# Kiripiro/leaffliction

Measured on AMD Instinct MI355X. Metric: 224x224 images/sec train, higher is better.
Workload: dtype f32; 1 GPU; leaf_cnn base train step (configs[1]: img 224, batch 256/GPU, fp32, 8 classes, AdamW+clipnorm+EMA, in-model augmentation); per_gpu_batch=256, global_batch=256, img_size=224, parallelism=dp1

## Files before the change

leaffliction_amd/csrc/lf_conv.hip:

```cpp
#include <type_traits>

#include "lf_common.h"

namespace {

typedef float f32x16 __attribute__((ext_vector_type(16)));
typedef float f32x4 __attribute__((ext_vector_type(4)));

constexpr int kThreads = 256;

typedef float lf_f4 __attribute__((ext_vector_type(4)));
constexpr unsigned kBufOob = 0xffffffffu;
__device__ __forceinline__ __amdgpu_buffer_rsrc_t buf_rsrc(const float* base, unsigned bytes) {
    return __builtin_amdgcn_make_buffer_rsrc(const_cast<float*>(base), 0, bytes, 0x00020000);
}
__device__ __forceinline__ float4 buf_load4(__amdgpu_buffer_rsrc_t r, unsigned off) {
    const lf_f4 v = __builtin_bit_cast(lf_f4, __builtin_amdgcn_raw_buffer_load_b128(r, off, 0, 0));
    return make_float4(v.x, v.y, v.z, v.w);
}
__device__ __forceinline__ float buf_load1(__amdgpu_buffer_rsrc_t r, unsigned off) {
    return __builtin_bit_cast(float, __builtin_amdgcn_raw_buffer_load_b32(r, off, 0, 0));
}

struct ConvArgs {
    const float* x;
    const float* w;
    const float* wino_u;
    float* y;
    const float* in_scale;
    const float* in_shift;
    int n, cin, cout, h, wd;
    int tiles_x, tiles_y;
    int in_relu;
    int accumulate;
    int vec_ok;
    int stack;
    float* stat_part;
    const float* stat_pivot;
    long long stat_tiles;
    const float* stat_mask_y;
    const float* mask_scale;
    const float* mask_shift;
    int mask_relu;
};

using lf::half_sum32;
using lf::pro_apply;
using lf::row_sum16;

__device__ __forceinline__ void wino_filter(const float (&g)[9], float (&u)[16]) {
    float t[4][3];
#pragma unroll
    for (int c = 0; c < 3; ++c) {
        const float s = g[c] + g[6 + c];
        t[0][c] = g[c];
        t[1][c] = (s + g[3 + c]) * 0.5f;
        t[2][c] = (s - g[3 + c]) * 0.5f;
        t[3][c] = g[6 + c];
    }
#pragma unroll
    for (int r = 0; r < 4; ++r) {
        const float s = t[r][0] + t[r][2];
        u[r * 4 + 0] = t[r][0];
        u[r * 4 + 1] = (s + t[r][1]) * 0.5f;
        u[r * 4 + 2] = (s - t[r][1]) * 0.5f;
        u[r * 4 + 3] = t[r][2];
    }
}
__device__ __forceinline__ void wino_input(const float (&d)[16], float (&v)[16]) {
    float t[16];
#pragma unroll
    for (int c = 0; c < 4; ++c) {
        t[0 + c] = d[0 + c] - d[8 + c];
        t[4 + c] = d[4 + c] + d[8 + c];
        t[8 + c] = d[8 + c] - d[4 + c];
        t[12 + c] = d[4 + c] - d[12 + c];
    }
#pragma unroll
    for (int r = 0; r < 4; ++r) {
        v[r * 4 + 0] = t[r * 4 + 0] - t[r * 4 + 2];
        v[r * 4 + 1] = t[r * 4 + 1] + t[r * 4 + 2];
        v[r * 4 + 2] = t[r * 4 + 2] - t[r * 4 + 1];
        v[r * 4 + 3] = t[r * 4 + 1] - t[r * 4 + 3];
    }
}
__device__ __forceinline__ void wino_output(const float (&m)[16], float (&y)[4]) {
    float b[2][4];
#pragma unroll
    for (int c = 0; c < 4; ++c) {
        b[0][c] = m[0 + c] + m[4 + c] + m[8 + c];
        b[1][c] = m[4 + c] - m[8 + c] - m[12 + c];
    }
#pragma unroll
    for (int r = 0; r < 2; ++r) {
        y[r * 2 + 0] = b[r][0] + b[r][1] + b[r][2];
        y[r * 2 + 1] = b[r][1] - b[r][2] - b[r][3];
    }
}

constexpr int kMaxProC = 512;

template <int TW, int TH, int HALO, bool STK>
struct ConvTile {
    int bz, by, tile;
    int tx0, ty0, n;
    int imgA, gyA0, ra;
    bool imgA_ok, imgB_ok;

    __device__ __forceinline__ explicit ConvTile(const ConvArgs& p) {
        const lf::Block3 b = lf::xcd_block3();
        bz = b.z;
        by = b.y;
        tile = b.x;
        tx0 = (tile % p.tiles_x) * TW;
        ty0 = (tile / p.tiles_x) * TH;
        n = bz * p.stack;
        imgA = ty0 / p.h;
        gyA0 = ty0 - imgA * p.h;
        ra = min(TH, p.h - gyA0);
        imgA_ok = imgA < p.stack && n + imgA < p.n;
        imgB_ok = STK && imgA + 1 < p.stack && n + imgA + 1 < p.n;
    }

    __device__ __forceinline__ bool patch_row(int py, int h, int& img, int& gy) const {
        if (py < ra + 2 * HALO) {
            img = imgA;
            gy = gyA0 - HALO + py;
            return imgA_ok && gy >= 0 && gy < h;
        }
        img = imgA + 1;
        gy = py - (ra + 2 * HALO) - HALO;
        return imgB_ok && ra < TH && gy >= 0 && gy < h && gy < TH - ra + HALO;
    }
};

template <int TW, int TH, int HALO, bool STK, int kKC>
struct PatchStage {
    static constexpr int PW = TW + 2 * HALO, PH = TH + 2 * HALO + (STK ? 2 * HALO : 0), PP = PW * PH;
    static constexpr int TW4 = TW / 4;
    static constexpr int NVI = kKC * PH * TW4, IPT = (NVI + kThreads - 1) / kThreads;
    static constexpr int NHI = kKC * PH * 2 * HALO, HPT = (NHI + kThreads - 1) / kThreads;
    static_assert(TW % 4 == 0, "float4 patch rows");

    size_t hw;
    float4 pv[IPT];
    float ph[HPT > 0 ? HPT : 1];
    unsigned pg[IPT], pl[IPT];
    unsigned hg[HPT > 0 ? HPT : 1], hl[HPT > 0 ? HPT : 1];
    unsigned okmask = 0;

    __device__ __forceinline__ PatchStage(const ConvArgs& p, const ConvTile<TW, TH, HALO, STK>& t, float* lsc, int tid) {
        if (p.in_scale != nullptr) {
            for (int c = tid; c < p.cin && c < kMaxProC; c += kThreads) {
                lsc[c] = p.in_scale[c];
                lsc[kMaxProC + c] = p.in_shift[c];
            }
        }
        hw = (size_t)p.h * p.wd;
        const unsigned uhw = (unsigned)hw;
#pragma unroll
        for (int i = 0; i < IPT; ++i) {
            const int e = tid + i * kThreads;
            const int kc = e / (PH * TW4), rem = e - kc * (PH * TW4);
            const int py = rem / TW4, slot = rem - py * TW4;
            int img, gy;
            const bool ok = t.patch_row(py, p.h, img, gy) && e < NVI;
            pg[i] = ok ? 4u * ((unsigned)(img * p.cin + kc) * uhw + (unsigned)gy * (unsigned)p.wd + (unsigned)(t.tx0 + 4 * slot)) : kBufOob;
            pl[i] = (unsigned)(kc * PP + py * PW + HALO + 4 * slot) | ((unsigned)kc << 16);
            okmask |= (ok ? 1u : 0u) << i;
        }
#pragma unroll
        for (int i = 0; i < HPT; ++i) {
            const int e = tid + i * kThreads;
            const int kc = e / (PH * 2), rem = e - kc * (PH * 2);
            const int py = rem >> 1, side = rem & 1;
            const int gx = side ? t.tx0 + TW : t.tx0 - 1;
            int img, gy;
            const bool ok = t.patch_row(py, p.h, img, gy) && e < NHI && gx >= 0 && gx < p.wd;
            hg[i] = ok ? 4u * ((unsigned)(img * p.cin + kc) * uhw + (unsigned)gy * (unsigned)p.wd + (unsigned)gx) : kBufOob;
            hl[i] = (unsigned)(kc * PP + py * PW + (side ? PW - 1 : 0)) | ((unsigned)kc << 16);
            okmask |= (ok ? 1u : 0u) << (16 + i);
        }
    }

    __device__ __forceinline__ void load(const ConvArgs& p, const float* xin, int c0) {
        const __amdgpu_buffer_rsrc_t rx = buf_rsrc(
            xin + (size_t)c0 * hw,
            4u * (unsigned)((STK ? (p.stack - 1) * p.cin : 0) + min(kKC, p.cin - c0)) * (unsigned)hw);
#pragma unroll
        for (int i = 0; i < IPT; ++i) pv[i] = buf_load4(rx, pg[i]);
#pragma unroll
        for (int i = 0; i < HPT; ++i) ph[i] = buf_load1(rx, hg[i]);
    }

    __device__ __forceinline__ void store(const ConvArgs& p, float* lp, const float* lsc, int c0, int tid) const {
        const bool pro = p.in_scale != nullptr;
        auto pro_sc = [&](int c) { return c < kMaxProC ? lsc[c] : p.in_scale[c]; };
        auto pro_sh = [&](int c) { return c < kMaxProC ? lsc[kMaxProC + c] : p.in_shift[c]; };
#pragma unroll
        for (int i = 0; i < IPT; ++i) {
            if (tid + i * kThreads < NVI) {
                const int kc = (int)(pl[i] >> 16);
                float4 v = pv[i];
                if (pro && (okmask >> i & 1u)) {
                    const float sc = pro_sc(c0 + kc), sh = pro_sh(c0 + kc);
                    v.x = pro_apply(v.x, sc, sh, p.in_relu);
                    v.y = pro_apply(v.y, sc, sh, p.in_relu);
                    v.z = pro_apply(v.z, sc, sh, p.in_relu);
                    v.w = pro_apply(v.w, sc, sh, p.in_relu);
                }
                float* dst = lp + (pl[i] & 0xffffu);
                dst[0] = v.x;
                dst[1] = v.y;
                dst[2] = v.z;
                dst[3] = v.w;
            }
        }
#pragma unroll
        for (int i = 0; i < HPT; ++i) {
            if (tid + i * kThreads < NHI) {
                const int kc = (int)(hl[i] >> 16);
                float v = ph[i];
                if (pro && (okmask >> (16 + i) & 1u))
                    v = pro_apply(v, pro_sc(c0 + kc), pro_sh(c0 + kc), p.in_relu);
                lp[hl[i] & 0xffffu] = v;
            }
        }
    }

    static __device__ __forceinline__ void stage_scalar(const ConvArgs& p, float* lp, const float* xin,
                                                        int tx0, int ty0, int c0, int tid) {
        constexpr int SLOTS = PP <= 64 ? 64 : (PP <= 128 ? 128 : 256);
        constexpr int G = kThreads / SLOTS;
        constexpr int ROUNDS = (PP + SLOTS - 1) / SLOTS;
        const int slot = tid % SLOTS, grp = tid / SLOTS;
        const size_t hw = (size_t)p.h * p.wd;
        const unsigned uhw = (unsigned)hw;
        const bool pro = p.in_scale != nullptr;
#pragma unroll
        for (int r = 0; r < ROUNDS; ++r) {
            const int pos = slot + r * SLOTS;
            if (pos < PP) {
                const int py = pos / PW, px = pos - py * PW;
                const int gy = ty0 + py - HALO, gx = tx0 + px - HALO;
                const bool inb = gy >= 0 && gy < p.h && gx >= 0 && gx < p.wd;
                const unsigned goff = inb ? (unsigned)gy * (unsigned)p.wd + (unsigned)gx : 0u;
#pragma unroll 4
                for (int kc = grp; kc < kKC; kc += G) {
                    const int c = c0 + kc;
                    float v = 0.f;
                    if (inb && c < p.cin) {
                        v = xin[(unsigned)c * uhw + goff];
                        if (pro) v = pro_apply(v, p.in_scale[c], p.in_shift[c], p.in_relu);
                    }
                    lp[kc * PP + pos] = v;
                }
            }
        }
    }
};

template <int WPX, int CT>
__device__ __forceinline__ void write_stat_part(const ConvArgs& p, const float* red, int bz, int tile, int co0,
                                                int tid) {
    __syncthreads();
    lf::write_stat_part<WPX, CT>(p.stat_part, p.stat_tiles, p.cout, (long long)bz * (p.tiles_x * p.tiles_y) + tile,
                                 co0, red, tid, kThreads);
}

template <int TAPS, int TW, int TH, int WCO, int MB, int WPX, int NB, int kKC, bool STK = false>
__global__ __launch_bounds__(kThreads, (MB * NB * 16 <= 32 ? 3 : 2))
void conv_mfma_kernel(ConvArgs p) {
    constexpr int NPB = TW * TH / 32;
    static_assert(TW * TH % 32 == 0, "tile must be whole 32-pixel blocks");
    static_assert(WCO * WPX == 4 && WPX * NB == NPB, "wave decomposition");
    constexpr int CT = 32 * WCO * MB;
    constexpr int HALO = TAPS == 9 ? 1 : 0;
    using Patch = PatchStage<TW, TH, HALO, STK, kKC>;
    constexpr int PW = Patch::PW, PP = Patch::PP;
    constexpr int PATCH = kKC * PP;
    constexpr int WSZ = kKC * TAPS * CT;
    static_assert(PATCH % 4 == 0, "16-byte aligned weight region");
    constexpr int CT4 = CT / 4, NWI = kKC * TAPS * CT4, WPT = (NWI + kThreads - 1) / kThreads;

    __shared__ __attribute__((aligned(16))) float lds[PATCH + WSZ];
    __shared__ float lsc[2 * kMaxProC];
    float* lp = lds;
    float* lw = lds + PATCH;

    const int tid = threadIdx.x, lane = tid & 63, wid = tid >> 6;
    const int wave_co = wid % WCO, wave_px = wid / WCO;
    const ConvTile<TW, TH, HALO, STK> t(p);
    const int co0 = t.by * CT;
    const size_t hw = (size_t)p.h * p.wd;
    const unsigned uhw = (unsigned)hw;
    const float* xin = p.x + (size_t)t.n * p.cin * hw;

    const int khalf = lane >> 5, j = lane & 31;
    int bbase[NB];
#pragma unroll
    for (int nb = 0; nb < NB; ++nb) {
        const int f = (wave_px * NB + nb) * 32 + j;
        const int r = f / TW, prow = (STK && r >= t.ra) ? r + 2 * HALO : r;
        bbase[nb] = khalf * PP + prow * PW + (f % TW);
    }
    const int abase = khalf * TAPS * CT + wave_co * MB * 32 + j;

    f32x16 acc[MB][NB];
#pragma unroll
    for (int m = 0; m < MB; ++m)
#pragma unroll
        for (int nb = 0; nb < NB; ++nb)
#pragma unroll
            for (int r = 0; r < 16; ++r) acc[m][nb][r] = 0.f;

    auto compute_chunk = [&]() {
#pragma unroll 2
        for (int cp = 0; cp < kKC / 2; ++cp) {
            const float* lwc = lw + abase + 2 * cp * TAPS * CT;
            const float* lpc = lp + 2 * cp * PP;
#pragma unroll
            for (int tap = 0; tap < TAPS; ++tap) {
                const int dy = TAPS == 9 ? tap / 3 : 0, dx = TAPS == 9 ? tap % 3 : 0;
                float a[MB], b[NB];
#pragma unroll
                for (int m = 0; m < MB; ++m) a[m] = lwc[tap * CT + m * 32];
#pragma unroll
                for (int nb = 0; nb < NB; ++nb) b[nb] = lpc[bbase[nb] + dy * PW + dx];
#pragma unroll
                for (int m = 0; m < MB; ++m)
#pragma unroll
                    for (int nb = 0; nb < NB; ++nb)
                        acc[m][nb] = __builtin_amdgcn_mfma_f32_32x32x2f32(a[m], b[nb], acc[m][nb], 0, 0, 0);
            }
        }
    };

    const int nchunks = (p.cin + kKC - 1) / kKC;
    const bool vec = p.vec_ok && (t.tx0 + TW <= p.wd);

    if (vec) {
        float4 wv[WPT];
        constexpr bool kPrefetchW = MB * NB * 16 <= 64;
        Patch patch(p, t, lsc, tid);
        unsigned wg[WPT];
#pragma unroll
        for (int i = 0; i < WPT; ++i) {
            const int e = tid + i * kThreads;
            const int row = e / CT4, col = (e - row * CT4) * 4;
            wg[i] = (e < NWI && co0 + col < p.cout) ? 4u * ((unsigned)row * (unsigned)p.cout + (unsigned)(co0 + col)) : kBufOob;
        }
        auto load_weights = [&](int c0) {
            const __amdgpu_buffer_rsrc_t rw =
                buf_rsrc(p.w + (size_t)c0 * TAPS * p.cout,
                         4u * (unsigned)(min(kKC, p.cin - c0) * TAPS) * (unsigned)p.cout);
#pragma unroll
            for (int i = 0; i < WPT; ++i) wv[i] = buf_load4(rw, wg[i]);
        };
        auto store_chunk = [&](int c0) {
            if (!kPrefetchW) load_weights(c0);
            patch.store(p, lp, lsc, c0, tid);
#pragma unroll
            for (int i = 0; i < WPT; ++i) {
                const int e = tid + i * kThreads;
                if (e < NWI) reinterpret_cast<float4*>(lw)[e] = wv[i];
            }
        };
        patch.load(p, xin, 0);
        if (kPrefetchW) load_weights(0);
        for (int ch = 0; ch < nchunks; ++ch) {
            __syncthreads();
            store_chunk(ch * kKC);
            __syncthreads();
            if (ch + 1 < nchunks) {
                patch.load(p, xin, (ch + 1) * kKC);
                if (kPrefetchW) load_weights((ch + 1) * kKC);
            }
            compute_chunk();
        }
    } else {
        constexpr int WROWS = kKC * TAPS, RPP = kThreads / CT;
        const int wcol = tid % CT, wrow0 = tid / CT;
        const bool wcol_ok = co0 + wcol < p.cout;
        for (int ch = 0; ch < nchunks; ++ch) {
            const int c0 = ch * kKC;
            __syncthreads();
            Patch::stage_scalar(p, lp, xin, t.tx0, t.ty0, c0, tid);
            const int wvalid = (p.cin - c0) * TAPS;
#pragma unroll 4
            for (int row = wrow0; row < WROWS; row += RPP) {
                float v = 0.f;
                if (wcol_ok && row < wvalid)
                    v = p.w[((unsigned)c0 * TAPS + row) * (unsigned)p.cout + (unsigned)(co0 + wcol)];
                lw[row * CT + wcol] = v;
            }
            __syncthreads();
            compute_chunk();
        }
    }

    float* yout = p.y + (size_t)t.n * p.cout * hw;
    const bool stats = p.stat_part != nullptr, masked = p.stat_mask_y != nullptr;
    float* red = lds;
    static_assert(WPX * CT * 2 <= PATCH + WSZ, "stat scratch must fit the staging LDS");
    if (stats) __syncthreads();
    const float* my = masked ? p.stat_mask_y + (size_t)t.n * p.cout * hw : nullptr;
    constexpr int RG = TAPS == 1 ? (NB <= 2 ? 4 : 1) : (NB <= 2 ? 16 : 4);
    bool pix_ok[NB];
    unsigned pixc[NB];
#pragma unroll
    for (int nb = 0; nb < NB; ++nb) {
        const int f = (wave_px * NB + nb) * 32 + j;
        const int r = f / TW, ox = t.tx0 + f % TW;
        const bool in_a = r < t.ra;
        const int oy = in_a ? t.gyA0 + r : r - t.ra;
        pix_ok[nb] = (in_a ? t.imgA_ok : t.imgB_ok) && oy < p.h && ox < p.wd;
        pixc[nb] = pix_ok[nb] ? (unsigned)((in_a ? t.imgA : t.imgA + 1) * p.cout) * uhw +
                                    (unsigned)oy * (unsigned)p.wd + (unsigned)ox
                              : 0u;
    }
#pragma unroll
    for (int m = 0; m < MB; ++m) {
#pragma unroll
        for (int rg = 0; rg < 16; rg += RG) {
            float oldv[RG][NB], yv[RG][NB];
            if (p.accumulate) {
#pragma unroll
                for (int rr = 0; rr < RG; ++rr) {
                    const int r = rg + rr;
                    const int co = co0 + (wave_co * MB + m) * 32 + 4 * khalf + (r & 3) + 8 * (r >> 2);
                    const float* src = yout + (size_t)min(co, p.cout - 1) * hw;
#pragma unroll
                    for (int nb = 0; nb < NB; ++nb) oldv[rr][nb] = src[pixc[nb]];
                }
            }
            if (masked) {
#pragma unroll
                for (int rr = 0; rr < RG; ++rr) {
                    const int r = rg + rr;
                    const int co = co0 + (wave_co * MB + m) * 32 + 4 * khalf + (r & 3) + 8 * (r >> 2);
                    const float* src = my + (size_t)min(co, p.cout - 1) * hw;
#pragma unroll
                    for (int nb = 0; nb < NB; ++nb) yv[rr][nb] = src[pixc[nb]];
                }
            }
#pragma unroll
            for (int rr = 0; rr < RG; ++rr) {
                const int r = rg + rr;
                const int cl = (wave_co * MB + m) * 32 + 4 * khalf + (r & 3) + 8 * (r >> 2);
                const int co = co0 + cl;
                const bool co_ok = co < p.cout;
                float* dst = yout + (size_t)co * hw;
#pragma unroll
                for (int nb = 0; nb < NB; ++nb) {
                    if (p.accumulate) acc[m][nb][r] += oldv[rr][nb];
                    if (co_ok && pix_ok[nb])
                        dst[pixc[nb]] = acc[m][nb][r];
                }
                if (!stats) continue;
                float s1 = 0.f, s2 = 0.f;
                if (!masked) {
                    const float pv = (p.stat_pivot != nullptr && co_ok) ? p.stat_pivot[co] : 0.f;
#pragma unroll
                    for (int nb = 0; nb < NB; ++nb)
                        lf::stat_accumulate(acc[m][nb][r], pix_ok[nb], false, pv, 0.f, 0.f, 0.f, 0, s1, s2);
                } else {
                    const float msc = p.mask_scale[min(co, p.cout - 1)], msh = p.mask_shift[min(co, p.cout - 1)];
#pragma unroll
                    for (int nb = 0; nb < NB; ++nb)
                        lf::stat_accumulate(acc[m][nb][r], co_ok && pix_ok[nb], true, 0.f, yv[rr][nb], msc, msh,
                                            p.mask_relu, s1, s2);
                }
                s1 = half_sum32(s1);
                s2 = half_sum32(s2);
                if (j == 31) {
                    red[(wave_px * CT + cl) * 2] = s1;
                    red[(wave_px * CT + cl) * 2 + 1] = s2;
                }
            }
        }
    }
    if (stats) write_stat_part<WPX, CT>(p, red, t.bz, t.tile, co0, tid);
}

template <int TW, int TH, int MB, int NB, bool STK>
__global__ __launch_bounds__(kThreads, 2)
void conv_wino_kernel(ConvArgs p) {
    constexpr int kKC = 8, WPX = 4;
    constexpr int TXN = TW / 2, NT = TXN * (TH / 2);
    static_assert(TH % 2 == 0, "F(2x2,3x3): even tile");
    static_assert(WPX * NB * 16 >= NT, "wave decomposition");
    constexpr int CT = 16 * MB;
    constexpr int kUP = 20;
    using Patch = PatchStage<TW, TH, 1, STK, kKC>;
    constexpr int PW = Patch::PW, PP = Patch::PP;
    constexpr int PATCH = kKC * PP;
    constexpr int WSZ = kKC * CT * kUP;
    static_assert(PATCH % 4 == 0, "16-byte aligned U region");

    __shared__ __attribute__((aligned(16))) float lds[PATCH + WSZ];
    __shared__ float lsc[2 * kMaxProC];
    float* lp = lds;
    float* lw = lds + PATCH;

    const int tid = threadIdx.x, lane = tid & 63, wave_px = tid >> 6;
    const ConvTile<TW, TH, 1, STK> t(p);
    const int co0 = t.by * CT;
    const size_t hw = (size_t)p.h * p.wd;
    const unsigned uhw = (unsigned)hw;
    const float* xin = p.x + (size_t)t.n * p.cin * hw;

    const int wq = lane >> 4, wl = lane & 15;
    int vbase[NB];
    const int ubase = (wq * CT + wl) * kUP;
    f32x4 wacc[MB][NB][16];
#pragma unroll
    for (int nb = 0; nb < NB; ++nb) {
        const int tt = min((wave_px * NB + nb) * 16 + wl, NT - 1);
        const int r0 = 2 * (tt / TXN), prow = (STK && r0 >= t.ra) ? r0 + 2 : r0;
        vbase[nb] = wq * PP + prow * PW + 2 * (tt % TXN);
    }
#pragma unroll
    for (int m = 0; m < MB; ++m)
#pragma unroll
        for (int nb = 0; nb < NB; ++nb)
#pragma unroll
            for (int q = 0; q < 16; ++q) wacc[m][nb][q] = f32x4{0.f, 0.f, 0.f, 0.f};

    auto compute_chunk = [&]() {
#pragma unroll
        for (int s = 0; s < kKC / 4; ++s) {
            float u[MB][16];
#pragma unroll
            for (int m = 0; m < MB; ++m) {
                const float4* us = reinterpret_cast<const float4*>(lw + ubase + (4 * s * CT + m * 16) * kUP);
#pragma unroll
                for (int q4 = 0; q4 < 4; ++q4) {
                    const float4 v4 = us[q4];
                    u[m][4 * q4 + 0] = v4.x;
                    u[m][4 * q4 + 1] = v4.y;
                    u[m][4 * q4 + 2] = v4.z;
                    u[m][4 * q4 + 3] = v4.w;
                }
            }
#pragma unroll
            for (int nb = 0; nb < NB; ++nb) {
                const float* src = lp + vbase[nb] + 4 * s * PP;
                float d[16], v[16];
#pragma unroll
                for (int r = 0; r < 4; ++r) {
                    const float2 lo = *reinterpret_cast<const float2*>(src + r * PW);
                    const float2 hi = *reinterpret_cast<const float2*>(src + r * PW + 2);
                    d[r * 4 + 0] = lo.x;
                    d[r * 4 + 1] = lo.y;
                    d[r * 4 + 2] = hi.x;
                    d[r * 4 + 3] = hi.y;
                }
                wino_input(d, v);
#pragma unroll
                for (int m = 0; m < MB; ++m)
#pragma unroll
                    for (int q = 0; q < 16; ++q)
                        wacc[m][nb][q] = __builtin_amdgcn_mfma_f32_16x16x4f32(u[m][q], v[q], wacc[m][nb][q], 0, 0, 0);
            }
        }
    };

    constexpr int KSTEP = kThreads / (4 * CT), UPT = kKC / KSTEP;
    static_assert(kThreads % (4 * CT) == 0 && kKC % KSTEP == 0, "whole channels per pass");
    const int ukc = tid / (4 * CT), uco = (tid >> 2) % CT, uq4 = tid & 3;
    const unsigned ustep = 64u * KSTEP * (unsigned)p.cout;
    const unsigned ugo = co0 + uco < p.cout ? 4u * (((unsigned)ukc * (unsigned)p.cout + (unsigned)(co0 + uco)) * 16u + 4u * (unsigned)uq4) : 0x80000000u;
    float* const ulds = lw + (ukc * CT + uco) * kUP + 4 * uq4;
    float4 uv[UPT];
    auto load_u = [&](int c0) {
        const __amdgpu_buffer_rsrc_t ru =
            buf_rsrc(p.wino_u + (size_t)c0 * p.cout * 16, 64u * (unsigned)min(kKC, p.cin - c0) * (unsigned)p.cout);
#pragma unroll
        for (int i = 0; i < UPT; ++i) uv[i] = buf_load4(ru, ugo + (unsigned)i * ustep);
    };
    auto store_u = [&]() {
#pragma unroll
        for (int i = 0; i < UPT; ++i) *reinterpret_cast<float4*>(ulds + i * KSTEP * CT * kUP) = uv[i];
    };

    const int nchunks = (p.cin + kKC - 1) / kKC;
    const bool vec = p.vec_ok && (t.tx0 + TW <= p.wd);

    if (vec) {
        Patch patch(p, t, lsc, tid);
        patch.load(p, xin, 0);
        for (int ch = 0; ch < nchunks; ++ch) {
            __syncthreads();
            load_u(ch * kKC);
            patch.store(p, lp, lsc, ch * kKC, tid);
            store_u();
            __syncthreads();
            if (ch + 1 < nchunks) patch.load(p, xin, (ch + 1) * kKC);
            compute_chunk();
        }
    } else {
        for (int ch = 0; ch < nchunks; ++ch) {
            const int c0 = ch * kKC;
            __syncthreads();
            Patch::stage_scalar(p, lp, xin, t.tx0, t.ty0, c0, tid);
            load_u(c0);
            store_u();
            __syncthreads();
            compute_chunk();
        }
    }

    float* yout = p.y + (size_t)t.n * p.cout * hw;
    const bool stats = p.stat_part != nullptr, masked = p.stat_mask_y != nullptr;
    float* red = lds;
    static_assert(WPX * CT * 2 <= PATCH + WSZ, "stat scratch must fit the staging LDS");
    if (stats) __syncthreads();
    const float* my = masked ? p.stat_mask_y + (size_t)t.n * p.cout * hw : nullptr;
    const bool y2 = (p.wd & 1) == 0 && (reinterpret_cast<size_t>(p.y) & 7) == 0;
    bool pok[NB][4];
    unsigned pofs[NB][4];
#pragma unroll
    for (int nb = 0; nb < NB; ++nb) {
        const int tt = (wave_px * NB + nb) * 16 + wl;
        const int r0 = 2 * (tt / TXN), ox = t.tx0 + 2 * (tt % TXN);
        const bool in_a = r0 < t.ra;
        const int oy = in_a ? t.gyA0 + r0 : r0 - t.ra;
        const bool img_ok = tt < NT && (in_a ? t.imgA_ok : t.imgB_ok);
        const unsigned base = (unsigned)((in_a ? t.imgA : t.imgA + 1) * p.cout) * uhw;
#pragma unroll
        for (int q = 0; q < 4; ++q) {
            const int py = oy + (q >> 1), px = ox + (q & 1);
            pok[nb][q] = img_ok && py < p.h && px < p.wd;
            pofs[nb][q] = pok[nb][q] ? base + (unsigned)py * (unsigned)p.wd + (unsigned)px : 0u;
        }
    }
#pragma unroll
    for (int m = 0; m < MB; ++m) {
#pragma unroll
        for (int i = 0; i < 4; ++i) {
            const int cl = m * 16 + 4 * wq + i;
            const int co = co0 + cl;
            const bool co_ok = co < p.cout;
            const size_t cofs = (size_t)min(co, p.cout - 1) * hw;
            float out[NB][4], oldv[NB][4], yv[NB][4];
#pragma unroll
            for (int nb = 0; nb < NB; ++nb) {
                float mm[16];
#pragma unroll
                for (int q = 0; q < 16; ++q) mm[q] = wacc[m][nb][q][i];
                wino_output(mm, out[nb]);
                if (p.accumulate) {
#pragma unroll
                    for (int q = 0; q < 4; ++q) oldv[nb][q] = yout[cofs + pofs[nb][q]];
                }
                if (masked) {
#pragma unroll
                    for (int q = 0; q < 4; ++q) yv[nb][q] = my[cofs + pofs[nb][q]];
                }
            }
#pragma unroll
            for (int nb = 0; nb < NB; ++nb) {
                if (p.accumulate) {
#pragma unroll
                    for (int q = 0; q < 4; ++q) out[nb][q] += oldv[nb][q];
                }
                if (co_ok) {
#pragma unroll
                    for (int r = 0; r < 2; ++r) {
                        float* dst = yout + cofs + pofs[nb][2 * r];
                        if (y2 && pok[nb][2 * r] && pok[nb][2 * r + 1]) {
                            *reinterpret_cast<float2*>(dst) = make_float2(out[nb][2 * r], out[nb][2 * r + 1]);
                        } else {
                            if (pok[nb][2 * r]) dst[0] = out[nb][2 * r];
                            if (pok[nb][2 * r + 1]) yout[cofs + pofs[nb][2 * r + 1]] = out[nb][2 * r + 1];
                        }
                    }
                }
            }
            if (!stats) continue;
            float s1 = 0.f, s2 = 0.f;
            if (!masked) {
                const float pv = (p.stat_pivot != nullptr && co_ok) ? p.stat_pivot[co] : 0.f;
#pragma unroll
                for (int nb = 0; nb < NB; ++nb)
#pragma unroll
                    for (int q = 0; q < 4; ++q)
                        lf::stat_accumulate(out[nb][q], pok[nb][q], false, pv, 0.f, 0.f, 0.f, 0, s1, s2);
            } else {
                const float msc = p.mask_scale[min(co, p.cout - 1)], msh = p.mask_shift[min(co, p.cout - 1)];
#pragma unroll
                for (int nb = 0; nb < NB; ++nb)
#pragma unroll
                    for (int q = 0; q < 4; ++q)
                        lf::stat_accumulate(out[nb][q], co_ok && pok[nb][q], true, 0.f, yv[nb][q], msc, msh, p.mask_relu,
                                            s1, s2);
            }
            s1 = row_sum16(s1);
            s2 = row_sum16(s2);
            if (wl == 0) {
                red[(wave_px * CT + cl) * 2] = s1;
                red[(wave_px * CT + cl) * 2 + 1] = s2;
            }
        }
    }
    if (stats) write_stat_part<WPX, CT>(p, red, t.bz, t.tile, co0, tid);
}

struct WgradArgs {
    const float* x;
    const float* dy;
    float* part;
    const float* in_scale;
    const float* in_shift;
    int n, cin, cout, h, wd;
    int tiles_x, tiles_y, items, items_per_split;
    int in_relu;
    int vec_ok;
    const float* bn_y;
    const float* bn_alpha;
    const float* bn_add;
    const float* bn_coef;
    float* dy_out;
    int bn_relu;
};

__device__ __forceinline__ float bn_dy1(float g, float y, float al, float ad, float c0, float c1,
                                        float c2, float c3, float c4, int relu) {
    float dz = fmaf(g, al, ad);
    if (relu && !(fmaf(y, c0, c1) > 0.f)) dz = 0.f;
    return fmaf(c2, dz, fmaf(c3, y, c4));
}

template <int TW, int TH, int WCI, int WCO, int KSPL>
__global__ __launch_bounds__(kThreads, 4) void wgrad_mfma_kernel(WgradArgs p) {
    static_assert(WCI * WCO * KSPL == 4, "wave decomposition");
    static_assert(TH % KSPL == 0 && TW % 4 == 0, "rows split across waves, float4 rows");
    constexpr int PP = (TW * TH) | 1;
    constexpr int CI_T = 32 * WCI, CO_T = 32 * WCO;
    constexpr int XSZ = CI_T * PP, DSZ = CO_T * PP;
    constexpr int RED = KSPL > 1 ? 1024 : 0;
    constexpr int LDSF = XSZ + DSZ > RED ? XSZ + DSZ : RED;
    constexpr int TW4 = TW / 4;
    constexpr int NXI = CI_T * TH * TW4, XPT = (NXI + kThreads - 1) / kThreads;
    constexpr int NDI = CO_T * TH * TW4, DPT = (NDI + kThreads - 1) / kThreads;
    __shared__ float lds[LDSF];
    float* lx = lds;
    float* ld = lds + XSZ;

    const int tid = threadIdx.x, lane = tid & 63, wid = tid >> 6;
    const int w_ci = wid % WCI, w_co = (wid / WCI) % WCO, w_k = wid / (WCI * WCO);
    const int ci0 = blockIdx.y * CI_T, co0 = blockIdx.z * CO_T;
    const int khalf = lane >> 5, j = lane & 31;
    const size_t hw = (size_t)p.h * p.wd;
    const unsigned uhw = (unsigned)hw;

    f32x16 acc;
#pragma unroll
    for (int r = 0; r < 16; ++r) acc[r] = 0.f;

    const int abase = (w_ci * 32 + j) * PP + khalf;
    const int bbase = (w_co * 32 + j) * PP + khalf;
    const bool pro = p.in_scale != nullptr;

    auto compute_item = [&]() {
        constexpr int ROWS = TH / KSPL;
#pragma unroll
        for (int rr = 0; rr < ROWS; ++rr) {
            const int row = w_k * ROWS + rr;
#pragma unroll 2
            for (int xx = 0; xx < TW; xx += 2) {
                const float b = ld[bbase + row * TW + xx];
                const float a = lx[abase + row * TW + xx];
                acc = __builtin_amdgcn_mfma_f32_32x32x2f32(a, b, acc, 0, 0, 0);
            }
        }
    };

    const int first = blockIdx.x * p.items_per_split;
    const int last = min(first + p.items_per_split, p.items);
    const int tiles = p.tiles_x * p.tiles_y;

    if (p.vec_ok) {
        float4 xv[XPT], dv[DPT];
        unsigned xok = 0;
        __shared__ float lsc[kMaxProC / 2];
        if (pro) {
            for (int c = tid; c < CI_T; c += kThreads) {
                const int gc = ci0 + c;
                lsc[c] = gc < p.cin ? p.in_scale[gc] : 1.f;
                lsc[kMaxProC / 4 + c] = gc < p.cin ? p.in_shift[gc] : 0.f;
            }
        }
        const bool bn = p.bn_y != nullptr;
        float4 yv[DPT];
        float dal[DPT], dad[DPT];
        unsigned dok = 0;
        __shared__ float lbn[5 * CO_T];
        if (bn) {
            for (int e = tid; e < 5 * CO_T; e += kThreads) {
                const int kk = e / CO_T, gc = co0 + (e - kk * CO_T);
                lbn[e] = gc < p.cout ? p.bn_coef[(size_t)kk * p.cout + gc] : 0.f;
            }
        }
        auto load_x = [&](int item) {
            const int n = item / tiles, t = item - n * tiles;
            const int tx0 = (t % p.tiles_x) * TW, ty0 = (t / p.tiles_x) * TH;
            const float* xin = p.x + (size_t)n * p.cin * hw;
            xok = 0;
#pragma unroll
            for (int i = 0; i < XPT; ++i) {
                const int e = tid + i * kThreads;
                float4 v = make_float4(0.f, 0.f, 0.f, 0.f);
                const int c = e / (TH * TW4), rem = e - c * (TH * TW4);
                const int py = rem / TW4, slot = rem - py * TW4;
                const int gc = ci0 + c, gy = ty0 + py;
                if (e < NXI && gc < p.cin && gy < p.h) {
                    v = *reinterpret_cast<const float4*>(xin + (unsigned)gc * uhw +
                                                         (unsigned)gy * (unsigned)p.wd + tx0 + 4 * slot);
                    xok |= 1u << i;
                }
                xv[i] = v;
            }
        };
        auto load_d = [&](int item) {
            const int n = item / tiles, t = item - n * tiles;
            const int tx0 = (t % p.tiles_x) * TW, ty0 = (t / p.tiles_x) * TH;
            const float* din = p.dy + (size_t)n * p.cout * hw;
            dok = 0;
#pragma unroll
            for (int i = 0; i < DPT; ++i) {
                const int e = tid + i * kThreads;
                float4 v = make_float4(0.f, 0.f, 0.f, 0.f);
                const int c = e / (TH * TW4), rem = e - c * (TH * TW4);
                const int py = rem / TW4, slot = rem - py * TW4;
                const int gc = co0 + c, gy = ty0 + py;
                if (e < NDI && gc < p.cout && gy < p.h) {
                    v = *reinterpret_cast<const float4*>(din + (unsigned)gc * uhw +
                                                         (unsigned)gy * (unsigned)p.wd + tx0 + 4 * slot);
                    dok |= 1u << i;
                }
                dv[i] = v;
            }
            if (bn) {
                const float* yin = p.bn_y + (size_t)n * p.cout * hw;
#pragma unroll
                for (int i = 0; i < DPT; ++i) {
                    const int e = tid + i * kThreads;
                    float4 v = make_float4(0.f, 0.f, 0.f, 0.f);
                    const int c = e / (TH * TW4), rem = e - c * (TH * TW4);
                    const int py = rem / TW4, slot = rem - py * TW4;
                    if (dok >> i & 1u)
                        v = *reinterpret_cast<const float4*>(yin + (unsigned)(co0 + c) * uhw +
                                                             (unsigned)(ty0 + py) * (unsigned)p.wd + tx0 + 4 * slot);
                    yv[i] = v;
                }
#pragma unroll
                for (int i = 0; i < DPT; ++i) {
                    const int gc = min(co0 + (tid + i * kThreads) / (TH * TW4), p.cout - 1);
                    dal[i] = p.bn_alpha != nullptr ? p.bn_alpha[(size_t)n * p.cout + gc] : 1.f;
                    dad[i] = p.bn_add != nullptr ? p.bn_add[(size_t)n * p.cout + gc] : 0.f;
                }
            }
        };
        auto store_x = [&]() {
#pragma unroll
            for (int i = 0; i < XPT; ++i) {
                const int e = tid + i * kThreads;
                if (e < NXI) {
                    const int c = e / (TH * TW4), rem = e - c * (TH * TW4);
                    const int py = rem / TW4, slot = rem - py * TW4;
                    float4 v = xv[i];
                    if (pro && (xok >> i & 1u)) {
                        const float sc = lsc[c], sh = lsc[kMaxProC / 4 + c];
                        v.x = pro_apply(v.x, sc, sh, p.in_relu);
                        v.y = pro_apply(v.y, sc, sh, p.in_relu);
                        v.z = pro_apply(v.z, sc, sh, p.in_relu);
                        v.w = pro_apply(v.w, sc, sh, p.in_relu);
                    }
                    float* dst = lx + c * PP + py * TW + 4 * slot;
                    dst[0] = v.x;
                    dst[1] = v.y;
                    dst[2] = v.z;
                    dst[3] = v.w;
                }
            }
        };
        auto store_d = [&](int item) {
            const int sn = item / tiles, st = item - sn * tiles;
            const int stx0 = (st % p.tiles_x) * TW, sty0 = (st / p.tiles_x) * TH;
#pragma unroll
            for (int i = 0; i < DPT; ++i) {
                const int e = tid + i * kThreads;
                if (e < NDI) {
                    const int c = e / (TH * TW4), rem = e - c * (TH * TW4);
                    float4 v = dv[i];
                    if (bn && (dok >> i & 1u)) {
                        const float c0 = lbn[c], c1 = lbn[CO_T + c], c2 = lbn[2 * CO_T + c],
                                    c3 = lbn[3 * CO_T + c], c4 = lbn[4 * CO_T + c];
                        v.x = bn_dy1(v.x, yv[i].x, dal[i], dad[i], c0, c1, c2, c3, c4, p.bn_relu);
                        v.y = bn_dy1(v.y, yv[i].y, dal[i], dad[i], c0, c1, c2, c3, c4, p.bn_relu);
                        v.z = bn_dy1(v.z, yv[i].z, dal[i], dad[i], c0, c1, c2, c3, c4, p.bn_relu);
                        v.w = bn_dy1(v.w, yv[i].w, dal[i], dad[i], c0, c1, c2, c3, c4, p.bn_relu);
                        if (blockIdx.y == 0 && p.dy_out != nullptr) {
                            const int py = rem / TW4, slot = rem - py * TW4;
                            *reinterpret_cast<float4*>(p.dy_out + ((size_t)sn * p.cout + co0 + c) * hw +
                                                       (size_t)(sty0 + py) * p.wd + stx0 + 4 * slot) = v;
                        }
                    }
                    float* dst = ld + c * PP + rem * 4;
                    dst[0] = v.x;
                    dst[1] = v.y;
                    dst[2] = v.z;
                    dst[3] = v.w;
                }
            }
        };
        if (first < last) {
            load_x(first);
            load_d(first);
        }
        for (int item = first; item < last; ++item) {
            __syncthreads();
            store_x();
            store_d(item);
            __syncthreads();
            if (item + 1 < last) {
                load_x(item + 1);
                load_d(item + 1);
            }
            compute_item();
        }
    } else {
        constexpr int POS = TW * TH;
        constexpr int SLOTS = POS <= 64 ? 64 : (POS <= 128 ? 128 : 256);
        constexpr int G = kThreads / SLOTS;
        static_assert(POS <= 256, "wgrad tiles are at most 256 positions");
        const int slot = tid % SLOTS, grp = tid / SLOTS;
        const int spy = slot / TW, spx = slot - spy * TW;
        for (int item = first; item < last; ++item) {
            const int n = item / tiles, t = item - n * tiles;
            const int tx0 = (t % p.tiles_x) * TW, ty0 = (t / p.tiles_x) * TH;
            const float* xin = p.x + (size_t)n * p.cin * hw;
            const float* din = p.dy + (size_t)n * p.cout * hw;
            __syncthreads();
            if (slot < POS) {
                const int gy = ty0 + spy, gx = tx0 + spx;
                const bool ok = gy < p.h && gx < p.wd;
                const unsigned off = ok ? (unsigned)gy * (unsigned)p.wd + (unsigned)gx : 0u;
#pragma unroll 4
                for (int c = grp; c < CI_T; c += G) {
                    const int gc = ci0 + c;
                    float v = 0.f;
                    if (ok && gc < p.cin) {
                        v = xin[(unsigned)gc * uhw + off];
                        if (pro) v = pro_apply(v, p.in_scale[gc], p.in_shift[gc], p.in_relu);
                    }
                    lx[c * PP + slot] = v;
                }
#pragma unroll 4
                for (int c = grp; c < CO_T; c += G) {
                    const int gc = co0 + c;
                    float v = 0.f;
                    if (ok && gc < p.cout) v = din[(unsigned)gc * uhw + off];
                    ld[c * PP + slot] = v;
                }
            }
            __syncthreads();
            compute_item();
        }
    }

    if (KSPL > 1) {
        const int q = w_co * WCI + w_ci;
#pragma unroll 1
        for (int k = 1; k < KSPL; ++k) {
#pragma unroll 1
            for (int qq = 0; qq < WCI * WCO; ++qq) {
                __syncthreads();
                if (w_k == k && q == qq) {
#pragma unroll
                    for (int r = 0; r < 16; ++r) lds[r * 64 + lane] = acc[r];
                }
                __syncthreads();
                if (w_k == 0 && q == qq) {
#pragma unroll
                    for (int r = 0; r < 16; ++r) acc[r] += lds[r * 64 + lane];
                }
            }
        }
    }
    if (w_k == 0) {
        float* out = p.part + (size_t)blockIdx.x * p.cin * p.cout;
        const int co = co0 + w_co * 32 + j;
#pragma unroll
        for (int r = 0; r < 16; ++r) {
            const int ci = ci0 + w_ci * 32 + (r & 3) + 8 * (r >> 2) + 4 * khalf;
            if (ci < p.cin && co < p.cout) out[(size_t)ci * p.cout + co] = acc[r];
        }
    }
}


template <int TW, int TH, int WCI, int WCO, int KSPL>
constexpr int wgrad3_lds_floats() {
    const int pp = ((TW + 2) * (TH + 2)) | 1, dp = (TW * TH) | 1;
    const int buf = 32 * WCI * pp + 32 * WCO * dp;
    const int red = KSPL > 1 ? 16 * 1024 : 0;
// ... 981 lines not shown
```

Baseline: 6184 images/sec.

## Stage per-channel stat constants in LDS and batch Winograd epilogue loads

```diff
diff --git a/leaffliction_amd/csrc/lf_conv.hip b/leaffliction_amd/csrc/lf_conv.hip
--- a/leaffliction_amd/csrc/lf_conv.hip
+++ b/leaffliction_amd/csrc/lf_conv.hip
@@ -100,6 +100,24 @@
 
 constexpr int kMaxProC = 512;
 
+template <int CT>
+__device__ __forceinline__ void stage_channel_consts(const ConvArgs& p, float* lsc, float* lep, int co0, int tid) {
+    static_assert(CT <= kThreads, "at most one cout per thread");
+    if (p.in_scale != nullptr) {
+        for (int c = tid; c < p.cin && c < kMaxProC; c += kThreads) {
+            lsc[c] = p.in_scale[c];
+            lsc[kMaxProC + c] = p.in_shift[c];
+        }
+    }
+    if (p.stat_part != nullptr && tid < CT) {
+        const int co = co0 + tid, coc = min(co, p.cout - 1);
+        const bool masked = p.stat_mask_y != nullptr;
+        lep[tid] = (!masked && p.stat_pivot != nullptr && co < p.cout) ? p.stat_pivot[co] : 0.f;
+        lep[CT + tid] = masked ? p.mask_scale[coc] : 0.f;
+        lep[2 * CT + tid] = masked ? p.mask_shift[coc] : 0.f;
+    }
+}
+
 template <int TW, int TH, int HALO, bool STK>
 struct ConvTile {
     int bz, by, tile;
@@ -149,13 +167,7 @@
     unsigned hg[HPT > 0 ? HPT : 1], hl[HPT > 0 ? HPT : 1];
     unsigned okmask = 0;
 
-    __device__ __forceinline__ PatchStage(const ConvArgs& p, const ConvTile<TW, TH, HALO, STK>& t, float* lsc, int tid) {
-        if (p.in_scale != nullptr) {
-            for (int c = tid; c < p.cin && c < kMaxProC; c += kThreads) {
-                lsc[c] = p.in_scale[c];
-                lsc[kMaxProC + c] = p.in_shift[c];
-            }
-        }
+    __device__ __forceinline__ PatchStage(const ConvArgs& p, const ConvTile<TW, TH, HALO, STK>& t, int tid) {
         hw = (size_t)p.h * p.wd;
         const unsigned uhw = (unsigned)hw;
 #pragma unroll
@@ -285,6 +297,7 @@
 
     __shared__ __attribute__((aligned(16))) float lds[PATCH + WSZ];
     __shared__ float lsc[2 * kMaxProC];
+    __shared__ float lep[3 * CT];
     float* lp = lds;
     float* lw = lds + PATCH;
 
@@ -342,7 +355,7 @@
     if (vec) {
         float4 wv[WPT];
         constexpr bool kPrefetchW = MB * NB * 16 <= 64;
-        Patch patch(p, t, lsc, tid);
+        Patch patch(p, t, tid);
         unsigned wg[WPT];
 #pragma unroll
         for (int i = 0; i < WPT; ++i) {
@@ -368,6 +381,7 @@
         };
         patch.load(p, xin, 0);
         if (kPrefetchW) load_weights(0);
+        stage_channel_consts<CT>(p, lsc, lep, co0, tid);
         for (int ch = 0; ch < nchunks; ++ch) {
             __syncthreads();
             store_chunk(ch * kKC);
@@ -382,6 +396,7 @@
         constexpr int WROWS = kKC * TAPS, RPP = kThreads / CT;
         const int wcol = tid % CT, wrow0 = tid / CT;
         const bool wcol_ok = co0 + wcol < p.cout;
+        stage_channel_consts<CT>(p, lsc, lep, co0, tid);
         for (int ch = 0; ch < nchunks; ++ch) {
             const int c0 = ch * kKC;
             __syncthreads();
@@ -423,6 +438,7 @@
     for (int m = 0; m < MB; ++m) {
 #pragma unroll
         for (int rg = 0; rg < 16; rg += RG) {
+            asm volatile("" ::: "memory");
             float oldv[RG][NB], yv[RG][NB];
             if (p.accumulate) {
 #pragma unroll
@@ -460,12 +476,12 @@
                 if (!stats) continue;
                 float s1 = 0.f, s2 = 0.f;
                 if (!masked) {
-                    const float pv = (p.stat_pivot != nullptr && co_ok) ? p.stat_pivot[co] : 0.f;
+                    const float pv = lep[cl];
 #pragma unroll
                     for (int nb = 0; nb < NB; ++nb)
                         lf::stat_accumulate(acc[m][nb][r], pix_ok[nb], false, pv, 0.f, 0.f, 0.f, 0, s1, s2);
                 } else {
-                    const float msc = p.mask_scale[min(co, p.cout - 1)], msh = p.mask_shift[min(co, p.cout - 1)];
+                    const float msc = lep[CT + cl], msh = lep[2 * CT + cl];
 #pragma unroll
                     for (int nb = 0; nb < NB; ++nb)
                         lf::stat_accumulate(acc[m][nb][r], co_ok && pix_ok[nb], true, 0.f, yv[rr][nb], msc, msh,
@@ -500,6 +516,7 @@
 
     __shared__ __attribute__((aligned(16))) float lds[PATCH + WSZ];
     __shared__ float lsc[2 * kMaxProC];
+    __shared__ float lep[3 * CT];
     float* lp = lds;
     float* lw = lds + PATCH;
 
@@ -588,11 +605,13 @@
     const bool vec = p.vec_ok && (t.tx0 + TW <= p.wd);
 
     if (vec) {
-        Patch patch(p, t, lsc, tid);
+        Patch patch(p, t, tid);
         patch.load(p, xin, 0);
+        load_u(0);
+        stage_channel_consts<CT>(p, lsc, lep, co0, tid);
         for (int ch = 0; ch < nchunks; ++ch) {
             __syncthreads();
-            load_u(ch * kKC);
+            if (ch > 0) load_u(ch * kKC);
             patch.store(p, lp, lsc, ch * kKC, tid);
             store_u();
             __syncthreads();
@@ -600,6 +619,7 @@
             compute_chunk();
         }
     } else {
+        stage_channel_consts<CT>(p, lsc, lep, co0, tid);
         for (int ch = 0; ch < nchunks; ++ch) {
             const int c0 = ch * kKC;
             __syncthreads();
@@ -617,9 +637,11 @@
     static_assert(WPX * CT * 2 <= PATCH + WSZ, "stat scratch must fit the staging LDS");
     if (stats) __syncthreads();
     const float* my = masked ? p.stat_mask_y + (size_t)t.n * p.cout * hw : nullptr;
-    const bool y2 = (p.wd & 1) == 0 && (reinterpret_cast<size_t>(p.y) & 7) == 0;
+    const bool y2 = (p.wd & 1) == 0 && (reinterpret_cast<size_t>(p.y) & 7) == 0 &&
+                    (reinterpret_cast<size_t>(p.stat_mask_y) & 7) == 0;
     bool pok[NB][4];
     unsigned pofs[NB][4];
+    bool lane_full = true;
 #pragma unroll
     for (int nb = 0; nb < NB; ++nb) {
         const int tt = (wave_px * NB + nb) * 16 + wl;
@@ -633,77 +655,111 @@
             const int py = oy + (q >> 1), px = ox + (q & 1);
             pok[nb][q] = img_ok && py < p.h && px < p.wd;
             pofs[nb][q] = pok[nb][q] ? base + (unsigned)py * (unsigned)p.wd + (unsigned)px : 0u;
-        }
-    }
-#pragma unroll
-    for (int m = 0; m < MB; ++m) {
-#pragma unroll
-        for (int i = 0; i < 4; ++i) {
-            const int cl = m * 16 + 4 * wq + i;
-            const int co = co0 + cl;
-            const bool co_ok = co < p.cout;
-            const size_t cofs = (size_t)min(co, p.cout - 1) * hw;
-            float out[NB][4], oldv[NB][4], yv[NB][4];
-#pragma unroll
-            for (int nb = 0; nb < NB; ++nb) {
-                float mm[16];
-#pragma unroll
-                for (int q = 0; q < 16; ++q) mm[q] = wacc[m][nb][q][i];
-                wino_output(mm, out[nb]);
-                if (p.accumulate) {
-#pragma unroll
-                    for (int q = 0; q < 4; ++q) oldv[nb][q] = yout[cofs + pofs[nb][q]];
-                }
-                if (masked) {
-#pragma unroll
-                    for (int q = 0; q < 4; ++q) yv[nb][q] = my[cofs + pofs[nb][q]];
-                }
-            }
-#pragma unroll
-            for (int nb = 0; nb < NB; ++nb) {
-                if (p.accumulate) {
-#pragma unroll
-                    for (int q = 0; q < 4; ++q) out[nb][q] += oldv[nb][q];
-                }
-                if (co_ok) {
-#pragma unroll
-                    for (int r = 0; r < 2; ++r) {
-                        float* dst = yout + cofs + pofs[nb][2 * r];
-                        if (y2 && pok[nb][2 * r] && pok[nb][2 * r + 1]) {
-                            *reinterpret_cast<float2*>(dst) = make_float2(out[nb][2 * r], out[nb][2 * r + 1]);
+            lane_full = lane_full && (pok[nb][q] || tt >= NT);
+        }
+    }
+    constexpr int STEPS = 4 * MB, G = (STEPS * NB <= 8 ? STEPS : 8 / NB);
+    static_assert(STEPS % G == 0, "whole groups");
+    auto epilogue = [&](auto full_c) {
+        constexpr bool FULL = decltype(full_c)::value;
+#pragma unroll
+        for (int g0 = 0; g0 < STEPS; g0 += G) {
+            float oldv[G][NB][4], yv[G][NB][4];
+            auto batch = [&](const float* src, float (&dst)[G][NB][4]) {
+#pragma unroll
+                for (int gs = 0; gs < G; ++gs) {
+                    const int m = (g0 + gs) / 4, i = (g0 + gs) % 4;
+                    const float* sp = src + (size_t)min(co0 + m * 16 + 4 * wq + i, p.cout - 1) * hw;
+#pragma unroll
+                    for (int nb = 0; nb < NB; ++nb) {
+                        if (FULL || y2) {
+#pragma unroll
+                            for (int r = 0; r < 2; ++r) {
+                                const float2 v2 = *reinterpret_cast<const float2*>(sp + pofs[nb][2 * r]);
+                                dst[gs][nb][2 * r] = v2.x;
+                                dst[gs][nb][2 * r + 1] = v2.y;
+                            }
                         } else {
-                            if (pok[nb][2 * r]) dst[0] = out[nb][2 * r];
-                            if (pok[nb][2 * r + 1]) yout[cofs + pofs[nb][2 * r + 1]] = out[nb][2 * r + 1];
+#pragma unroll
+                            for (int q = 0; q < 4; ++q) dst[gs][nb][q] = sp[pofs[nb][q]];
                         }
                     }
                 }
-            }
-            if (!stats) continue;
-            float s1 = 0.f, s2 = 0.f;
-            if (!masked) {
-                const float pv = (p.stat_pivot != nullptr && co_ok) ? p.stat_pivot[co] : 0.f;
-#pragma unroll
-                for (int nb = 0; nb < NB; ++nb)
-#pragma unroll
-                    for (int q = 0; q < 4; ++q)
-                        lf::stat_accumulate(out[nb][q], pok[nb][q], false, pv, 0.f, 0.f, 0.f, 0, s1, s2);
-            } else {
-                const float msc = p.mask_scale[min(co, p.cout - 1)], msh = p.mask_shift[min(co, p.cout - 1)];
-#pragma unroll
-                for (int nb = 0; nb < NB; ++nb)
-#pragma unroll
-                    for (int q = 0; q < 4; ++q)
-                        lf::stat_accumulate(out[nb][q], co_ok && pok[nb][q], true, 0.f, yv[nb][q], msc, msh, p.mask_relu,
-                                            s1, s2);
-            }
-            s1 = row_sum16(s1);
-            s2 = row_sum16(s2);
-            if (wl == 0) {
-                red[(wave_px * CT + cl) * 2] = s1;
-                red[(wave_px * CT + cl) * 2 + 1] = s2;
-            }
-        }
-    }
+            };
+            if (p.accumulate) batch(yout, oldv);
+            if (masked) batch(my, yv);
+#pragma unroll
+            for (int gs = 0; gs < G; ++gs) {
+                const int m = (g0 + gs) / 4, i = (g0 + gs) % 4;
+                const int cl = m * 16 + 4 * wq + i;
+                const int co = co0 + cl;
+                const bool co_ok = FULL || co < p.cout;
+                const size_t cofs = (size_t)min(co, p.cout - 1) * hw;
+                float out[NB][4];
+#pragma unroll
+                for (int nb = 0; nb < NB; ++nb) {
+                    float mm[16];
+#pragma unroll
+                    for (int q = 0; q < 16; ++q) mm[q] = wacc[m][nb][q][i];
+                    wino_output(mm, out[nb]);
+                }
+#pragma unroll
+                for (int nb = 0; nb < NB; ++nb) {
+                    if (p.accumulate) {
+#pragma unroll
+                        for (int q = 0; q < 4; ++q) out[nb][q] += oldv[gs][nb][q];
+                    }
+                    if (FULL) {
+                        if (NT == WPX * NB * 16 || pok[nb][0]) {
+#pragma unroll
+                            for (int r = 0; r < 2; ++r)
+                                *reinterpret_cast<float2*>(yout + cofs + pofs[nb][2 * r]) =
+                                    make_float2(out[nb][2 * r], out[nb][2 * r + 1]);
+                        }
+                    } else if (co_ok) {
+#pragma unroll
+                        for (int r = 0; r < 2; ++r) {
+                            float* dst = yout + cofs + pofs[nb][2 * r];
+                            if (y2 && pok[nb][2 * r] && pok[nb][2 * r + 1]) {
+                                *reinterpret_cast<float2*>(dst) = make_float2(out[nb][2 * r], out[nb][2 * r + 1]);
+                            } else {
+                                if (pok[nb][2 * r]) dst[0] = out[nb][2 * r];
+                                if (pok[nb][2 * r + 1]) yout[cofs + pofs[nb][2 * r + 1]] = out[nb][2 * r + 1];
+                            }
+                        }
+                    }
+                }
+                if (!stats) continue;
+                float s1 = 0.f, s2 = 0.f;
+                if (!masked) {
+                    const float pv = lep[cl];
+#pragma unroll
+                    for (int nb = 0; nb < NB; ++nb)
+#pragma unroll
+                        for (int q = 0; q < 4; ++q)
+                            lf::stat_accumulate(out[nb][q], pok[nb][q], false, pv, 0.f, 0.f, 0.f, 0, s1, s2);
+                } else {
+                    const float msc = lep[CT + cl], msh = lep[2 * CT + cl];
+#pragma unroll
+                    for (int nb = 0; nb < NB; ++nb)
+#pragma unroll
+                        for (int q = 0; q < 4; ++q)
+                            lf::stat_accumulate(out[nb][q], co_ok && pok[nb][q], true, 0.f, yv[gs][nb][q], msc, msh,
+                                                p.mask_relu, s1, s2);
+                }
+                s1 = row_sum16(s1);
+                s2 = row_sum16(s2);
+                if (wl == 0) {
+                    red[(wave_px * CT + cl) * 2] = s1;
+                    red[(wave_px * CT + cl) * 2 + 1] = s2;
+                }
+            }
+        }
+    };
+    if (__all(y2 && lane_full && co0 + CT <= p.cout))
+        epilogue(std::true_type{});
+    else
+        epilogue(std::false_type{});
     if (stats) write_stat_part<WPX, CT>(p, red, t.bz, t.tile, co0, tid);
 }
 
```

Result: faster. 6487 images/sec (median of 6 runs) (+4.9%).
